# JohannesBuchner/massivedatans

Measured on AMD Instinct MI355X. Metric: likelihood evals/sec across N datasets per constrained draw, higher is better.
Workload: dtype f64

## Files before the change

### massivedatans_amd/csrc/mdns_core.hip

```cpp
#include "mdns_internal.h"
#include <time.h>

#include <atomic>
#include <cmath>
#include <cstdarg>
#include <cstdio>
#include <cstdlib>
#include <cstring>
#include <mutex>
#include <vector>

namespace mdns {

static char g_error[512] = "";

void set_error(const char *fmt, ...)
{
	va_list ap;
	va_start(ap, fmt);
	vsnprintf(g_error, sizeof(g_error), fmt, ap);
	va_end(ap);
	if (getenv("MDNS_VERBOSE")) fprintf(stderr, "[mdns] %s\n", g_error);
}

// ... 33 lines not shown
	if (device >= count) {
		set_error("device %d requested but only %d visible", device, count);
		return 1;
	}
	if (g_ctx_ready) {
		set_error("mdns_init(%d): this process already runs on device %d; one process drives one GPU "
		          "(start one process per GPU)", device, g_ctx.device);
		return 1;
	}
	if (!MDNS_HIP(hipSetDevice(device))) return 1;
	hipDeviceProp_t prop;
	if (!MDNS_HIP(hipGetDeviceProperties(&prop, device))) return 1;
	g_ctx.device = device;
	g_ctx.num_cus = prop.multiProcessorCount > 0 ? prop.multiProcessorCount : 256;
	if (!MDNS_HIP(hipStreamCreateWithFlags(&g_ctx.own_stream, hipStreamNonBlocking))) return 1;
	g_ctx.stream = g_ctx.own_stream;
	g_ctx_ready = true;
	return 0;
}

Context *ctx()
{
	std::lock_guard<std::mutex> lock(g_ctx_mutex);
	if (!g_ctx_ready && init_locked(-1) != 0) return nullptr;
	(void) hipSetDevice(g_ctx.device);
	return &g_ctx;
}

void *device_scratch(size_t bytes)
{
	Context *c = ctx();
	if (!c) return nullptr;
	if (bytes <= c->d_ws_bytes) return c->d_ws;
	if (c->d_ws) {
		(void) hipStreamSynchronize(c->stream);
		(void) hipFree(c->d_ws);
		c->d_ws = nullptr; c->d_ws_bytes = 0;
	}
	size_t cap = bytes + bytes / 2 + 4096;
	if (!MDNS_HIP(hipMalloc(&c->d_ws, cap))) return nullptr;
	c->d_ws_bytes = cap;
	return c->d_ws;
}

void *mask_scratch(size_t bytes)
{
	Context *c = ctx();
	if (!c) return nullptr;
	if (bytes <= c->d_mask_bytes) return c->d_mask;
	if (c->d_mask) {
		(void) hipStreamSynchronize(c->stream);
		(void) hipFree(c->d_mask);
		c->d_mask = nullptr; c->d_mask_bytes = 0;
	}
	size_t cap = bytes + bytes / 2 + 4096;
	if (!MDNS_HIP(hipMalloc(&c->d_mask, cap))) return nullptr;
	c->d_mask_bytes = cap;
	return c->d_mask;
}

void *pinned_scratch(size_t bytes)
{
	Context *c = ctx();
	if (!c) return nullptr;
	if (bytes <= c->h_pin_bytes) return c->h_pin;
// ... 46 lines not shown

static void drain_pending()
{
	for (TimedLaunch &t : g_pending) {
		float ms = 0;
		if (hipEventSynchronize(t.stop) == hipSuccess && hipEventElapsedTime(&ms, t.start, t.stop) == hipSuccess) {
			g_prof_count[t.which] += 1;
			g_prof_ms[t.which] += ms;
		}
		g_event_pool.push_back(t.start);
		g_event_pool.push_back(t.stop);
	}
	g_pending.clear();
}

ProfileScope::ProfileScope(int which) : slot(-1)
{
	if (!(g_profiling & (1 << which)) || !g_ctx_ready) return;
	if (g_prof_seen[which]++ % g_prof_every != 0) return;
	TimedLaunch t{which, pooled_event(), pooled_event()};
	if (!t.start || !t.stop) return;
	(void) hipEventRecord(t.start, g_ctx.stream);
	g_pending.push_back(t);
	slot = (int) g_pending.size() - 1;
}

ProfileScope::~ProfileScope()
{
	if (slot < 0) return;
	(void) hipEventRecord(g_pending[slot].stop, g_ctx.stream);
	if (g_pending.size() >= 4096) drain_pending();
}

template <typename T>
static bool grow(T **p, size_t *cap, size_t need)
{
	if (need <= *cap) return true;
	Context *c = ctx();
	if (!c) return false;
	if (*p) { (void) hipStreamSynchronize(c->stream); (void) hipFree(*p); *p = nullptr; *cap = 0; }
	size_t n = need + need / 2 + 64;
	if (!MDNS_HIP(hipMalloc((void **) p, n * sizeof(T)))) return false;
	*cap = n;
	return true;
}
// ... 13 lines not shown
}

extern "C" int mdns_init(int device)
{
	std::lock_guard<std::mutex> lock(g_ctx_mutex);
	return init_locked(device);
}

extern "C" void *mdns_dev_alloc(size_t bytes)
{
	if (!ctx()) return nullptr;
	void *p = nullptr;
	if (!MDNS_HIP(hipMalloc(&p, bytes ? bytes : 8))) return nullptr;
	return p;
}
extern "C" void mdns_dev_free(void *p) { if (p && ctx()) (void) hipFree(p); }
extern "C" int mdns_h2d(void *dst, const void *src, size_t bytes)
{
	Context *c = ctx();
	if (!c) return 1;
	if (!MDNS_HIP(hipMemcpyAsync(dst, src, bytes, hipMemcpyHostToDevice, c->stream))) return 1;
	return MDNS_HIP(hipStreamSynchronize(c->stream)) ? 0 : 1;
}
extern "C" int mdns_d2h(void *dst, const void *src, size_t bytes)
{
	Context *c = ctx();
	if (!c) return 1;
	if (!MDNS_HIP(hipMemcpyAsync(dst, src, bytes, hipMemcpyDeviceToHost, c->stream))) return 1;
	return MDNS_HIP(hipStreamSynchronize(c->stream)) ? 0 : 1;
}
extern "C" int mdns_d2d(void *dst, const void *src, size_t bytes)
{
	Context *c = ctx();
	if (!c) return 1;
	return MDNS_HIP(hipMemcpyAsync(dst, src, bytes, hipMemcpyDeviceToDevice, c->stream)) ? 0 : 1;
}
extern "C" int mdns_sync(void)
{
	Context *c = ctx();
	if (!c) return 1;
	return MDNS_HIP(hipStreamSynchronize(c->stream)) ? 0 : 1;
}
extern "C" int mdns_set_stream(void *hip_stream)
{
	Context *c = ctx();
	if (!c) return 1;
	c->stream = hip_stream ? (hipStream_t) hip_stream : c->own_stream;
	return 0;
}
extern "C" void *mdns_get_stream(void)
{
	Context *c = ctx();
	return c ? (void *) c->stream : nullptr;
}
extern "C" void *mdns_event_create(void)
{
	if (!ctx()) return nullptr;
	hipEvent_t ev;
	if (!MDNS_HIP(hipEventCreate(&ev))) return nullptr;
	return (void *) ev;
}
extern "C" void mdns_event_destroy(void *ev) { if (ev) (void) hipEventDestroy((hipEvent_t) ev); }
extern "C" int mdns_event_record(void *ev)
{
	Context *c = ctx();
	if (!c || !ev) return 1;
	return MDNS_HIP(hipEventRecord((hipEvent_t) ev, c->stream)) ? 0 : 1;
}
extern "C" double mdns_event_elapsed_ms(void *a, void *b)
{
	if (!a || !b) return NAN;
	if (!MDNS_HIP(hipEventSynchronize((hipEvent_t) b))) return NAN;
	float ms = 0;
	if (!MDNS_HIP(hipEventElapsedTime(&ms, (hipEvent_t) a, (hipEvent_t) b))) return NAN;
	return (double) ms;
}

extern "C" int mdns_profile(int classes)
{
	if (!ctx()) return 1;
	drain_pending();
// ... 341 lines not shown
	if (temporary) mdns_spectra_destroy(s);
	if (rc != 0) return rc;
	double *Lout = (double *) Loutp;
	for (int k = 0; k < M; k++) Lout[rows[k]] = L[k];
	return 0;
}

extern "C" int mdns_count_within_dev(const double *d_members, int K, int ndim, double maxdistance,
                                     const double *d_cands, int M, int *d_counts)
{
	Context *c = ctx();
	if (!c) return 1;
	if (K < 0 || M < 0 || ndim <= 0) { set_error("mdns_count_within_dev: bad sizes"); return 1; }
	if (M == 0) return 0;
	if (K == 0) return MDNS_HIP(hipMemsetAsync(d_counts, 0, (size_t) M * sizeof(int), c->stream)) ? 0 : 1;
	return launch_count_within(d_members, K, ndim, sqrt_threshold(maxdistance), nullptr, d_cands, M, d_counts) ? 0 : 1;
}

extern "C" int mdns_bootstrap_round_maxsq_dev(const double *d_members, int K, int ndim,
                                              const double *d_chosen, int nbootstraps,
                                              double *d_round_sq)
{
	Context *c = ctx();
	if (!c) return 1;
	if (K < 0 || nbootstraps < 0 || ndim <= 0) { set_error("mdns_bootstrap_round_maxsq_dev: bad sizes"); return 1; }
	if (nbootstraps == 0) return 0;
	if (K == 0) return MDNS_HIP(hipMemsetAsync(d_round_sq, 0, (size_t) nbootstraps * sizeof(double), c->stream)) ? 0 : 1;
	return launch_bootstrap(d_members, K, ndim, d_chosen, nbootstraps, d_round_sq) ? 0 : 1;
}

static bool stage_in(const void *const *src, const size_t *bytes, int n, size_t extra_bytes, char **d_ptrs,
                     char **d_extra)
{
	Context *c = ctx();
	size_t total = 0;
	for (int i = 0; i < n; i++) total += (bytes[i] + 255) & ~(size_t) 255;
	char *base = (char *) device_scratch(total + extra_bytes + 256);
	if (!base) return false;
	size_t off = 0;
	for (int i = 0; i < n; i++) {
		d_ptrs[i] = base + off;
		if (bytes[i] && !MDNS_HIP(hipMemcpyAsync(d_ptrs[i], src[i], bytes[i], hipMemcpyHostToDevice, c->stream)))
			return false;
// ... 145 lines not shown
			void *p = g_pool[i].p;
			g_pool[i] = g_pool.back();
			g_pool.pop_back();
			*got = want;
			return p;
		}
	void *p = nullptr;
	if (!MDNS_HIP(hipMalloc(&p, want))) return nullptr;
	*got = want;
	return p;
}

static void pool_give(void *p, size_t bytes)
{
	if (!p) return;
	if (g_pool.size() >= 64) { (void) hipFree(p); return; }
	g_pool.push_back({bytes, p});
}

static bool pool_fit(void **p, size_t *cap, size_t need)
{
	if (need <= *cap) return true;
	pool_give(*p, *cap);
	*cap = 0;
	*p = pool_take(need, cap);
	return *p != nullptr;
}

static bool region_fetch(mdns_region *r);

static bool poll_expired(long long *started_ns)
{
	static const double limit_s = [] { const char *v = getenv("MDNS_POLL_TIMEOUT_S"); const double t = v ? atof(v) : 120.0; return t > 0 ? t : 120.0; }();
	struct timespec ts;
	clock_gettime(CLOCK_MONOTONIC, &ts);
	const long long now = (long long) ts.tv_sec * 1000000000LL + ts.tv_nsec;
	if (*started_ns == 0) { *started_ns = now; return false; }
	return (double) (now - *started_ns) * 1e-9 > limit_s;
}

Wait mdns::wait_seq(const volatile unsigned long long *at, unsigned long long want, hipError_t *err)
{
	long long started = 0;
	for (unsigned spin = 0; *at != want; spin++) {
		if ((spin & 1023) != 1023) continue;
		const hipError_t e = hipStreamQuery(g_ctx.stream);
		if (e == hipErrorNotReady) {
			if (poll_expired(&started)) return Wait::timeout;
			continue;
		}
		if (e != hipSuccess) {
			if (err) *err = e;
			return Wait::failed;
		}
		if (*at != want) return Wait::empty;
	}
	std::atomic_thread_fence(std::memory_order_acquire);
	return Wait::ok;
}

template <class Choice>
static bool region_launch_radius(mdns_region *r, bool (*launch)(const double *, int, int, const Choice *, int, double *, const BootstrapFinish *),
                                 const Choice *d_choice, int nbootstraps)
{
	const BootstrapFinish fin = {r->d_counter, r->d_res, r->h_res_dev, ++r->seq};
	if (!launch(r->d_members, r->K, r->ndim, d_choice, nbootstraps, r->d_round, &fin)) return false;
	r->on_device = true;
	r->pending = true;
	return true;
}

static mdns_region *region_new(const double *d_members, double *owned, int K, int ndim)
{
	mdns_region *r = new mdns_region();
	r->d_members = d_members; r->owned = owned; r->K = K; r->ndim = ndim;
	r->slot = take_result_slot();
	if (r->slot < 0) { mdns_region_destroy(r); return nullptr; }
	const ResultSlab &slab = g_slabs[r->slot / kSlabSlots];
	const int i = r->slot % kSlabSlots;
	r->d_res = slab.d_res + i;
	r->d_counter = slab.d_counter + i;
// ... 13 lines not shown
	const size_t bytes = (size_t) K * ndim * sizeof(double);
	size_t got = 0;
	double *d = (double *) pool_take(bytes, &got);
	if (!d) return nullptr;
	if (!MDNS_HIP(hipMemcpyAsync(d, members, bytes, hipMemcpyHostToDevice, c->stream)) ||
	    !MDNS_HIP(hipStreamSynchronize(c->stream))) { pool_give(d, got); return nullptr; }
	mdns_region *r = region_new(d, d, K, ndim);
	if (r) r->owned_bytes = got; else pool_give(d, got);
	return r;
}

static mdns_region *create_bootstrapped(const double *members, int K, int ndim, const unsigned *packed, int nbootstraps,
                                        double *radius, bool wait)
{
	Context *c = ctx();
	if (!c) return nullptr;
	if (!members || !packed || (wait && !radius) || K <= 0 || ndim <= 0 || nbootstraps <= 0 || nbootstraps > 16) {
		set_error("mdns_region_create_bootstrapped: bad arguments (K=%d ndim=%d rounds=%d)", K, ndim, nbootstraps);
		return nullptr;
	}
	const size_t mbytes = (size_t) K * ndim * sizeof(double), pbytes = (size_t) K * sizeof(unsigned);
	const size_t poff = (mbytes + 255) & ~(size_t) 255;
	size_t got = 0;
	char *d = (char *) pool_take(poff + pbytes, &got);
	if (!d) return nullptr;
	char *pin = (char *) pinned_scratch(poff + pbytes);
	if (!pin) { pool_give(d, got); return nullptr; }
	memcpy(pin, members, mbytes);
	memcpy(pin + poff, packed, pbytes);
	if (!MDNS_HIP(hipMemcpyAsync(d, pin, poff + pbytes, hipMemcpyHostToDevice, c->stream))) { pool_give(d, got); return nullptr; }
	mdns_region *r = region_new((const double *) d, (double *) d, K, ndim);
	if (!r) { (void) hipStreamSynchronize(c->stream); pool_give(d, got); return nullptr; }
	r->owned_bytes = got;
	if (!region_launch_radius(r, launch_bootstrap_packed, (const unsigned *) (d + poff), nbootstraps)) {
		(void) hipStreamSynchronize(c->stream);
		mdns_region_destroy(r);
		return nullptr;
	}
	if (!wait) return r;
	*radius = mdns_region_radius(r);
	if (*radius != *radius) { mdns_region_destroy(r); return nullptr; }
	return r;
}

extern "C" mdns_region *mdns_region_create_bootstrapped(const double *members, int K, int ndim,
                                                        const unsigned *packed, int nbootstraps, double *radius)
{
	return create_bootstrapped(members, K, ndim, packed, nbootstraps, radius, true);
}

mdns_region *mdns::region_begin_bootstrapped(const double *members, int K, int ndim, const unsigned *packed, int nbootstraps)
{
	return create_bootstrapped(members, K, ndim, packed, nbootstraps, nullptr, false);
}

bool mdns::region_view(mdns_region *r, RegionView *out)
{
	if (!r || !out || !r->on_device) return false;
	out->d_members = r->d_members; out->K = r->K; out->ndim = r->ndim; out->d_res = r->d_res;
	return true;
}

extern "C" mdns_region *mdns_region_wrap_dev(const double *d_members, int K, int ndim)
{
	if (!ctx()) return nullptr;
	if (!d_members || K <= 0 || ndim <= 0) { set_error("mdns_region_wrap_dev: bad arguments"); return nullptr; }
	return region_new(d_members, nullptr, K, ndim);
}

extern "C" void mdns_region_destroy(mdns_region *r)
{
	if (!r) return;
	if (r->pending && ctx()) (void) region_fetch(r);
	pool_give(r->owned, r->owned_bytes);
	pool_give(r->own_round, r->own_round_bytes);
	pool_give(r->d_chosen, r->chosen_bytes);
	pool_give(r->d_points, r->points_bytes);
	pool_give(r->d_counts, r->counts_bytes);
	if (r->slot >= 0) g_free_slots.push_back(r->slot);
	delete r;
}

extern "C" int mdns_region_set_radius(mdns_region *r, double maxdistance)
{
	if (!r) { set_error("null region"); return 1; }
	if (r->pending && ctx()) (void) region_fetch(r);
	r->radius = maxdistance;
	r->thresh_sq = sqrt_threshold(maxdistance);
	r->on_device = false;
	r->pending = false;
	return 0;
}

static bool region_fetch(mdns_region *r)
{
	if (!r->pending) return true;
	hipError_t e = hipSuccess;
	switch (wait_seq(&r->h_res->seq, r->seq, &e)) {
	case Wait::ok: break;
	case Wait::timeout: set_error("radius computation: no result within MDNS_POLL_TIMEOUT_S"); return false;
	case Wait::failed: set_error("radius computation failed: %s", hipGetErrorString(e)); return false;
	case Wait::empty: set_error("radius computation finished without a result"); return false;
	}
	r->radius = r->h_res->radius;
	r->thresh_sq = sqrt_threshold(r->radius);
	r->pending = false;
	return true;
}

extern "C" double mdns_region_radius(mdns_region *r)
{
	if (!r || !ctx() || !region_fetch(r)) return NAN;
	return r->radius;
}

extern "C" int mdns_region_bootstrap_radius_async(mdns_region *r, const double *d_chosen, int nbootstraps)
{
	Context *c = ctx();
	if (!c || !r) return 1;
	if (nbootstraps <= 0) { set_error("mdns_region_bootstrap_radius: nbootstraps=%d", nbootstraps); return 1; }
	if (!region_fetch(r)) return 1;
	if (r->round_cap < nbootstraps) {
		if (!pool_fit((void **) &r->own_round, &r->own_round_bytes, (size_t) nbootstraps * sizeof(double))) return 1;
		r->d_round = r->own_round;
		if (!MDNS_HIP(hipMemsetAsync(r->d_round, 0, (size_t) nbootstraps * sizeof(double), c->stream))) return 1;
		r->round_cap = nbootstraps;
	}
	return region_launch_radius(r, launch_bootstrap, d_chosen, nbootstraps) ? 0 : 1;
}

extern "C" double mdns_region_bootstrap_radius_dev(mdns_region *r, const double *d_chosen, int nbootstraps)
{
	if (mdns_region_bootstrap_radius_async(r, d_chosen, nbootstraps) != 0) return NAN;
	return mdns_region_radius(r);
}

extern "C" double mdns_region_bootstrap_radius(mdns_region *r, const double *chosen, int nbootstraps)
{
	Context *c = ctx();
	if (!c || !r) return NAN;
	const size_t n = (size_t) r->K * (nbootstraps > 0 ? nbootstraps : 0);
	if (n == 0) { set_error("mdns_region_bootstrap_radius: nbootstraps=%d", nbootstraps); return NAN; }
	if (!pool_fit(&r->d_chosen, &r->chosen_bytes, n * sizeof(double))) return NAN;
	if (!MDNS_HIP(hipMemcpyAsync(r->d_chosen, chosen, n * sizeof(double), hipMemcpyHostToDevice, c->stream))) return NAN;
	return mdns_region_bootstrap_radius_dev(r, (const double *) r->d_chosen, nbootstraps);
}

extern "C" double mdns_region_bootstrap_radius_packed(mdns_region *r, const unsigned *packed, int nbootstraps)
{
	Context *c = ctx();
	if (!c || !r) return NAN;
	if (nbootstraps <= 0 || nbootstraps > 16 || !packed) { set_error("mdns_region_bootstrap_radius_packed: nbootstraps=%d (1..16)", nbootstraps); return NAN; }
	if (!region_fetch(r)) return NAN;
	const size_t bytes = (size_t) r->K * sizeof(unsigned);
	if (!pool_fit(&r->d_chosen, &r->chosen_bytes, bytes)) return NAN;
	if (!MDNS_HIP(hipMemcpyAsync(r->d_chosen, packed, bytes, hipMemcpyHostToDevice, c->stream))) return NAN;
	if (!region_launch_radius(r, launch_bootstrap_packed, (const unsigned *) r->d_chosen, nbootstraps)) return NAN;
	return mdns_region_radius(r);
}

extern "C" int mdns_region_count_dev(mdns_region *r, const double *d_points, int M, int *d_counts)
{
	if (!ctx() || !r) return 1;
	if (M < 0) { set_error("mdns_region_count: M=%d", M); return 1; }
	if (M == 0) return 0;
	if (!r->on_device && r->radius != r->radius) { set_error("mdns_region_count: the region has no radius yet"); return 1; }
	return launch_count_within(r->d_members, r->K, r->ndim, r->thresh_sq, r->on_device ? r->d_res : nullptr,
	                           d_points, M, d_counts) ? 0 : 1;
}

static char *g_stage = nullptr, *g_stage_dev = nullptr;
static size_t g_stage_points = 0, g_stage_doubles = 0;
static unsigned long long g_stage_seq = 0;
static int *g_stage_ticket = nullptr;

extern "C" int mdns_region_count_polled(mdns_region *r, const double *points, int M, int *counts)
{
	Context *c = ctx();
	if (!c || !r) return 1;
	if (M <= 0) return M < 0;
	if (!r->on_device && r->radius != r->radius) { set_error("mdns_region_count: the region has no radius yet"); return 1; }
	const size_t n = (size_t) M * r->ndim;
	if ((size_t) M > g_stage_points || n > g_stage_doubles) {
		if (g_stage) { (void) hipStreamSynchronize(c->stream); (void) hipHostFree(g_stage); g_stage = nullptr; }
		const size_t np = (size_t) M + M / 2 + 1024, nd = n + n / 2 + 4096;
		if (!MDNS_HIP(hipHostMalloc((void **) &g_stage, 64 + np * sizeof(int) + 64 + nd * sizeof(double), hipHostMallocMapped)) ||
		    !MDNS_HIP(hipHostGetDevicePointer((void **) &g_stage_dev, g_stage, 0))) { g_stage = nullptr; g_stage_points = g_stage_doubles = 0; return 1; }
		g_stage_points = np; g_stage_doubles = nd;
		*(volatile unsigned long long *) g_stage = g_stage_seq;
	}
	if (!g_stage_ticket) {
		if (!MDNS_HIP(hipMalloc((void **) &g_stage_ticket, sizeof(int))) ||
		    !MDNS_HIP(hipMemsetAsync(g_stage_ticket, 0, sizeof(int), c->stream))) { g_stage_ticket = nullptr; return 1; }
	}
	const size_t off_counts = 64, off_points = (64 + g_stage_points * sizeof(int) + 63) & ~(size_t) 63;
	memcpy(g_stage + off_points, points, n * sizeof(double));
	const unsigned long long seq = ++g_stage_seq;
	const CountMail mail = {g_stage_ticket, (unsigned long long *) g_stage_dev, seq};
	if (!launch_count_within(r->d_members, r->K, r->ndim, r->thresh_sq, r->on_device ? r->d_res : nullptr,
	                         (const double *) (g_stage_dev + off_points), M, (int *) (g_stage_dev + off_counts), &mail)) return 1;
	hipError_t e = hipSuccess;
	switch (wait_seq((const volatile unsigned long long *) g_stage, seq, &e)) {
	case Wait::ok: break;
	case Wait::timeout: set_error("membership count: no result within MDNS_POLL_TIMEOUT_S"); return 1;
	case Wait::failed: set_error("membership count failed: %s", hipGetErrorString(e)); return 1;
	case Wait::empty:
		(void) hipMemsetAsync(g_stage_ticket, 0, sizeof(int), c->stream);
		set_error("membership count finished without a result");
		return 1;
	}
	memcpy(counts, g_stage + off_counts, (size_t) M * sizeof(int));
	return 0;
}

extern "C" int mdns_region_count(mdns_region *r, const double *points, int M, int *counts)
{
	Context *c = ctx();
	if (!c || !r) return 1;
	if (M <= 0) return M < 0;
	const size_t n = (size_t) M * r->ndim;
	if (!pool_fit(&r->d_points, &r->points_bytes, n * sizeof(double)) ||
	    !pool_fit(&r->d_counts, &r->counts_bytes, (size_t) M * sizeof(int))) return 1;
	if (!MDNS_HIP(hipMemcpyAsync(r->d_points, points, n * sizeof(double), hipMemcpyHostToDevice, c->stream))) return 1;
	if (mdns_region_count_dev(r, (const double *) r->d_points, M, (int *) r->d_counts) != 0) return 1;
	if (!MDNS_HIP(hipMemcpyAsync(counts, r->d_counts, (size_t) M * sizeof(int), hipMemcpyDeviceToHost, c->stream))) return 1;
	return MDNS_HIP(hipStreamSynchronize(c->stream)) ? 0 : 1;
}
```

### massivedatans_amd/csrc/mdns_internal.h

```cpp
#pragma once
#include <hip/hip_runtime.h>
#include <cstddef>
#include <cstdint>
#include "mdns.h"

namespace mdns {

void set_error(const char *fmt, ...);
bool hip_ok(hipError_t e, const char *what, const char *file, int line);
#define MDNS_HIP(call) ::mdns::hip_ok((call), #call, __FILE__, __LINE__)
bool launched(const char *name);

enum class Wait { ok, timeout, failed, empty };
Wait wait_seq(const volatile unsigned long long *at, unsigned long long want, hipError_t *err = nullptr);

struct Context {
	int device = -1;
	hipStream_t own_stream = nullptr;
	hipStream_t stream = nullptr;
	int num_cus = 256;
	void *d_ws = nullptr;   size_t d_ws_bytes = 0;
	void *h_pin = nullptr;  size_t h_pin_bytes = 0;
	void *d_mask = nullptr; size_t d_mask_bytes = 0;
};
Context *ctx();
void *device_scratch(size_t bytes);
void *pinned_scratch(size_t bytes);
void *mask_scratch(size_t bytes);

}

struct mdns_spectra {
	int ndata = 0;
	int nx = 0;
	int ld = 0;
	double *d_y = nullptr;
	double *d_yT = nullptr;
	int ldT = 0;
	double *d_w = nullptr;
	double *d_x = nullptr;
// ... 103 lines not shown
	double radius;
	double thresh;
	unsigned long long seq;
	unsigned long long pad;
};
struct BootstrapFinish {
	unsigned *counter;
	RegionResult *d_res;
	RegionResult *h_res;
	unsigned long long seq;
};

mdns_region *region_begin_bootstrapped(const double *members, int K, int ndim, const unsigned *packed, int nbootstraps);

struct CountMail { int *ticket; unsigned long long *seq_at; unsigned long long seq; };
bool launch_count_within(const double *d_members, int K, int ndim, double thresh_sq,
                         const RegionResult *d_res, const double *d_cands, int M, int *d_counts,
                         const CountMail *mail = nullptr);
bool launch_bootstrap(const double *d_members, int K, int ndim, const double *d_chosen,
                      int nbootstraps, double *d_round_sq, const BootstrapFinish *finish = nullptr);
bool launch_bootstrap_packed(const double *d_members, int K, int ndim, const unsigned *d_packed,
                             int nbootstraps, double *d_round_sq, const BootstrapFinish *finish);
bool launch_nn_maxsq(const double *d_members, int K, int ndim, double *d_out);
bool bootstrap_sorted_applies(int K, int ndim, int nbootstraps);
bool launch_bootstrap_sorted(const double *d_members, int K, int ndim, const unsigned *d_packed, int nbootstraps,
                             double *d_round_sq, const BootstrapFinish *finish);

struct RegionView { const double *d_members; int K, ndim; const RegionResult *d_res; };
bool region_view(mdns_region *r, RegionView *out);
static constexpr int kChainMost = 1024;
static constexpr int kChainDim = 8;
struct ChainSpec {
	int n, ndim, nparams, limit, identity;
	double mn[kChainDim], mx[kChainDim];
// ... 4 lines not shown
struct ChainBox {
	unsigned long long seq;
	int nkept, B;
	int counts[kChainMost];
	double params[kChainMost][3];
	double u[kChainMost * kChainDim];
};
bool launch_box_count(const RegionView &rv, const ChainSpec &spec, ChainBox *box_dev, double *d_props, int *d_counts,
                      const CountMail *mail);
bool launch_chain_accept(const mdns_spectra *s, const ChainSpec &spec, const double *d_props, const int *d_counts,
                         ChainBox *box_dev, double scale, const int *d_rows_in, int *d_rows_dev, int M,
                         const double *d_higher, int *d_flags, int stamp, const JointTrail &trail, void *d_header);

struct ProfileScope {
	int slot;
	explicit ProfileScope(int which);
	~ProfileScope();
};
void note_kernel(int which, const char *fmt, ...);

#ifdef __HIPCC__
__device__ __forceinline__ void handover_release()
{
	__builtin_amdgcn_fence(__ATOMIC_RELEASE, "workgroup");
	asm volatile("s_waitcnt vmcnt(0)" ::: "memory");
}
__device__ __forceinline__ void handover_acquire() { __builtin_amdgcn_fence(__ATOMIC_ACQUIRE, "workgroup"); }
template <class T, class V> __device__ __forceinline__ void mail_store(T *at, V v) { __hip_atomic_store(at, (T) v, __ATOMIC_RELAXED, __HIP_MEMORY_SCOPE_SYSTEM); }
__device__ __forceinline__ void mail_raise(unsigned long long *seq_at, unsigned long long seq) { handover_release(); mail_store(seq_at, seq); }

template <int U>
// ... 119 lines not shown
```

### massivedatans_amd/csrc/mdns_neighbors.hip

```cpp
#include "mdns_geom.h"
#include <cstdlib>
#include <cstring>

#pragma clang fp contract(off)

namespace mdns {

static constexpr int kBlock = 256;
static constexpr int kMaxTile = 512;
static constexpr int kRounds = 16;
static constexpr size_t kLdsBudget = 60 * 1024;

template <int SL> struct Geo {
	static constexpr int PTS = 64 / SL;
	static constexpr int NSLICE = 4 * SL;
};

template <typename T>
__device__ __forceinline__ void stage_to_lds(T *__restrict__ dst, const T *__restrict__ src, int count)
{
	constexpr int U = 8;
	for (int base = 0; base < count; base += U * kBlock) {
		T r[U];
#pragma unroll
// ... 253 lines not shown
{
	__shared__ double wmax[4][RT];
	merge_chunks<RT, false>(part, K, ny, blockIdx.x * (kBlock / 4), mask, nb, round_sq, wmax);
	finish_radius(fin, round_sq, nround_all);
}

static int pick_tile(int ndim, size_t per_member_extra, size_t fixed_bytes)
{
	const size_t per = (size_t) ndim * sizeof(double) + per_member_extra;
	if (fixed_bytes + 16 * per > kLdsBudget) return 0;
	size_t n = (kLdsBudget - fixed_bytes) / per;
	if (n > (size_t) kMaxTile) n = kMaxTile;
	return (int) (n & ~(size_t) 15);
}

bool launch_count_within(const double *d_members, int K, int ndim, double thresh_sq,
                         const RegionResult *d_res, const double *d_cands, int M, int *d_counts, const CountMail *mail)
{
	Context *c = ctx();
	const CountMail none = {nullptr, nullptr, 0};
	const CountMail post = mail ? *mail : none;
	const size_t fixed = 4 * 64 * sizeof(int);
	const int tile_n = pick_tile(ndim, 0, fixed);
	if (tile_n <= 0) { set_error("ndim=%d too large for the member tile", ndim); return false; }
	const bool small = (M + 63) / 64 < 2 * c->num_cus;
	const bool fine = mail != nullptr && small;
	const int pts = fine ? 4 : (small ? 16 : 64);
	const int gx = (M + pts - 1) / pts;
	int want = (2 * c->num_cus + gx - 1) / gx;
	int max_split = (K + tile_n - 1) / tile_n;
	int gy = want < max_split ? want : max_split;
	if (mail) gy = 1;
	if (gy < 1) gy = 1;
	if (gy > 65535) gy = 65535;
	int kchunk = (K + gy - 1) / gy;
	kchunk = ((kchunk + tile_n - 1) / tile_n) * tile_n;
	gy = (K + kchunk - 1) / kchunk;
	const int accumulate = gy > 1 ? 1 : 0;
	if (accumulate && !MDNS_HIP(hipMemsetAsync(d_counts, 0, (size_t) M * sizeof(int), c->stream))) return false;
	const size_t lds = (size_t) tile_n * ndim * sizeof(double) + fixed;
	dim3 grid(gx, gy);
	ProfileScope prof(2);
#define COUNT_LAUNCH(D) do { if (fine) hipLaunchKernelGGL((k_count_within<D, 16>), grid, dim3(kBlock), lds, c->stream, \
		d_members, K, ndim, thresh_sq, d_res, d_cands, M, d_counts, kchunk, tile_n, accumulate, post); \
	else if (small) hipLaunchKernelGGL((k_count_within<D, 4>), grid, dim3(kBlock), lds, c->stream, \
		d_members, K, ndim, thresh_sq, d_res, d_cands, M, d_counts, kchunk, tile_n, accumulate, post); \
	else hipLaunchKernelGGL((k_count_within<D, 1>), grid, dim3(kBlock), lds, c->stream, \
		d_members, K, ndim, thresh_sq, d_res, d_cands, M, d_counts, kchunk, tile_n, accumulate, post); } while (0)
	MDNS_DIM_SWITCH(ndim, COUNT_LAUNCH)
#undef COUNT_LAUNCH
	return launched("k_count_within");
}

template <bool NN>
static bool launch_nearest(const double *d_members, int K, int ndim, const double *d_chosen,
                           int nboot, double *d_round_sq, const BootstrapFinish *finish,
                           const unsigned *d_packed = nullptr)
{
	Context *c = ctx();
	const bool small = (K + 63) / 64 < 2 * c->num_cus;
	const size_t fixed = (size_t) 4 * (NN ? 1 : (nboot > 10 ? kRounds : 10)) * (small ? 16 : 64) * sizeof(double);
	const int tile_n = pick_tile(ndim, sizeof(unsigned), fixed);
	if (tile_n <= 0) { set_error("ndim=%d too large for the member tile", ndim); return false; }
	const size_t lds = (size_t) tile_n * ndim * sizeof(double) + fixed + (size_t) tile_n * sizeof(unsigned);
	unsigned *d_mask = const_cast<unsigned *>(d_packed);
	if (!NN && !d_packed) {
		d_mask = (unsigned *) mask_scratch((size_t) K * sizeof(unsigned));
		if (!d_mask) return false;
	}
	const bool fused = !NN && finish && K <= 2048 && !d_packed;
	const int pts = small ? 16 : 64;
	dim3 grid((K + pts - 1) / pts);
	for (int b0 = 0; b0 < nboot; b0 += kRounds) {
		const int nb = nboot - b0 < kRounds ? nboot - b0 : kRounds;
		if (!NN && !fused && !d_packed) {
			const int nthreads = K > nb ? K : nb;
			hipLaunchKernelGGL(k_pack_chosen, dim3((nthreads + kBlock - 1) / kBlock), dim3(kBlock), 0, c->stream,
			                   d_chosen, K, nboot, b0, nb, d_mask, d_round_sq);
			if (!launched("k_pack_chosen")) return false;
		}
		BootstrapFinish fin = {nullptr, nullptr, nullptr, 0};
		if (finish && b0 + kRounds >= nboot) fin = *finish;
		ProfileScope prof(3);
#define NEAR_LAUNCH_R(D, SL, RT) hipLaunchKernelGGL((k_nearest_chosen<D, NN, SL, RT>), grid, dim3(kBlock), lds, c->stream, \
		d_members, K, ndim, d_mask, nb, d_round_sq + b0, tile_n, fin, d_round_sq, nboot, fused ? d_chosen : nullptr, nboot, b0)
#define NEAR_LAUNCH(D) do { \
	if (small) { if (NN || nb <= 10) NEAR_LAUNCH_R(D, 4, 10); else NEAR_LAUNCH_R(D, 4, kRounds); } \
	else       { if (NN || nb <= 10) NEAR_LAUNCH_R(D, 1, 10); else NEAR_LAUNCH_R(D, 1, kRounds); } } while (0)
		MDNS_DIM_SWITCH(ndim, NEAR_LAUNCH)
#undef NEAR_LAUNCH
#undef NEAR_LAUNCH_R
		if (!launched("k_nearest_chosen")) return false;
	}
	return true;
}

bool launch_bootstrap(const double *d_members, int K, int ndim, const double *d_chosen,
                      int nbootstraps, double *d_round_sq, const BootstrapFinish *finish)
{
	return launch_nearest<false>(d_members, K, ndim, d_chosen, nbootstraps, d_round_sq, finish);
}

static int uniform_chunks(int K)
{
	int most = K / 128;
	if (most < 1) most = 1;
	int best = most < 16 ? most : 16;
	static const char *forced = getenv("MDNS_K6_GY");
	if (forced && atoi(forced) > 0) best = atoi(forced) < most ? atoi(forced) : most;
	return best;
}

bool launch_bootstrap_packed(const double *d_members, int K, int ndim, const unsigned *d_packed,
                             int nbootstraps, double *d_round_sq, const BootstrapFinish *finish)
{
// ... 29 lines not shown
			    !MDNS_HIP(hipMemsetAsync(d_tickets, 0, (size_t) cap * sizeof(unsigned), c->stream))) { d_tickets = nullptr; tickets_cap = 0; return false; }
			tickets_cap = cap;
		}
		unsigned *tickets = fold ? d_tickets : nullptr;
#define UNI_LAUNCH(D) do { if (rt == 10) hipLaunchKernelGGL((k_nearest_uniform<D, 10>), grid, dim3(kBlock), lds, c->stream, d_members, K, d_packed, kchunk, tile_n, d_part, tickets, nbootstraps, d_round_sq, *finish, nbootstraps); \
		else hipLaunchKernelGGL((k_nearest_uniform<D, kRounds>), grid, dim3(kBlock), lds, c->stream, d_members, K, d_packed, kchunk, tile_n, d_part, tickets, nbootstraps, d_round_sq, *finish, nbootstraps); } while (0)
		MDNS_DIM5_SWITCH(ndim, UNI_LAUNCH)
#undef UNI_LAUNCH
		if (!launched("k_nearest_uniform")) return false;
		if (fold) return true;
		const dim3 fgrid((K + kBlock / 4 - 1) / (kBlock / 4));
		if (rt == 10) hipLaunchKernelGGL((k_nearest_finish<10>), fgrid, dim3(kBlock), 0, c->stream, (const double *) d_part, K, ny, d_packed, nbootstraps, d_round_sq, *finish, nbootstraps);
		else hipLaunchKernelGGL((k_nearest_finish<kRounds>), fgrid, dim3(kBlock), 0, c->stream, (const double *) d_part, K, ny, d_packed, nbootstraps, d_round_sq, *finish, nbootstraps);
		return launched("k_nearest_finish");
	}
	return launch_nearest<false>(d_members, K, ndim, nullptr, nbootstraps, d_round_sq, finish, d_packed);
}

bool launch_nn_maxsq(const double *d_members, int K, int ndim, double *d_out)
{
	return launch_nearest<true>(d_members, K, ndim, nullptr, 1, d_out, nullptr);
}

}
```

Measured before the change: 28.38 billion.

## Run async region bootstrap and count kernels on a side stream with fork/join events

Adds a second non-blocking stream plus fork/join events so the async region radius bootstrap and device-side count launches can run beside work on the main stream. The fork is skipped when no other context entry happened since the last fork, and every synchronous entry point, copy, free and region access joins the side stream first. The aim is to overlap region kernels with other GPU work and to avoid serialising them behind the main stream. The cost is extra bookkeeping, event waits and new ordering hazards, for example an entry point that forgets to join.

```diff
diff --git a/massivedatans_amd/csrc/mdns_core.hip b/massivedatans_amd/csrc/mdns_core.hip
--- a/massivedatans_amd/csrc/mdns_core.hip
+++ b/massivedatans_amd/csrc/mdns_core.hip
@@ -71,17 +71,46 @@
 	g_ctx.device = device;
 	g_ctx.num_cus = prop.multiProcessorCount > 0 ? prop.multiProcessorCount : 256;
 	if (!MDNS_HIP(hipStreamCreateWithFlags(&g_ctx.own_stream, hipStreamNonBlocking))) return 1;
+	if (!MDNS_HIP(hipStreamCreateWithFlags(&g_ctx.region_stream, hipStreamNonBlocking))) return 1;
+	if (!MDNS_HIP(hipEventCreateWithFlags(&g_ctx.fork_event, hipEventDisableTiming))) return 1;
+	if (!MDNS_HIP(hipEventCreateWithFlags(&g_ctx.join_event, hipEventDisableTiming))) return 1;
 	g_ctx.stream = g_ctx.own_stream;
 	g_ctx_ready = true;
 	return 0;
 }
 
-Context *ctx()
+static Context *ctx_entered(bool counts)
 {
 	std::lock_guard<std::mutex> lock(g_ctx_mutex);
 	if (!g_ctx_ready && init_locked(-1) != 0) return nullptr;
 	(void) hipSetDevice(g_ctx.device);
+	if (counts) g_ctx.entered++;
 	return &g_ctx;
+}
+
+Context *ctx() { return ctx_entered(true); }
+
+static hipStream_t region_fork(Context *c)
+{
+	if (c->stream != c->own_stream) return c->stream;
+	if (c->entered != c->forked_at || c->stream_lent) {
+		if (!MDNS_HIP(hipEventRecord(c->fork_event, c->own_stream)) ||
+		    !MDNS_HIP(hipStreamWaitEvent(c->region_stream, c->fork_event, 0))) return nullptr;
+	}
+	c->region_busy = true;
+	return c->region_stream;
+}
+static void region_forked(Context *c, hipStream_t on) { if (on == c->region_stream) c->forked_at = c->entered; }
+
+bool region_join(Context *c)
+{
+	if (!c->region_busy) return true;
+	c->region_busy = false;
+	return MDNS_HIP(hipEventRecord(c->join_event, c->region_stream)) && MDNS_HIP(hipStreamWaitEvent(c->stream, c->join_event, 0));
+}
+static void region_drain(Context *c)
+{
+	if (c->region_busy) (void) hipStreamSynchronize(c->region_stream);
 }
 
 void *device_scratch(size_t bytes)
@@ -106,6 +135,7 @@
 	if (!c) return nullptr;
 	if (bytes <= c->d_mask_bytes) return c->d_mask;
 	if (c->d_mask) {
+		region_drain(c);
 		(void) hipStreamSynchronize(c->stream);
 		(void) hipFree(c->d_mask);
 		c->d_mask = nullptr; c->d_mask_bytes = 0;
@@ -182,13 +212,13 @@
 	g_pending.clear();
 }
 
-ProfileScope::ProfileScope(int which) : slot(-1)
+ProfileScope::ProfileScope(int which, hipStream_t on_) : slot(-1), on(on_ ? on_ : g_ctx.stream)
 {
 	if (!(g_profiling & (1 << which)) || !g_ctx_ready) return;
 	if (g_prof_seen[which]++ % g_prof_every != 0) return;
 	TimedLaunch t{which, pooled_event(), pooled_event()};
 	if (!t.start || !t.stop) return;
-	(void) hipEventRecord(t.start, g_ctx.stream);
+	(void) hipEventRecord(t.start, on);
 	g_pending.push_back(t);
 	slot = (int) g_pending.size() - 1;
 }
@@ -196,7 +226,7 @@
 ProfileScope::~ProfileScope()
 {
 	if (slot < 0) return;
-	(void) hipEventRecord(g_pending[slot].stop, g_ctx.stream);
+	(void) hipEventRecord(g_pending[slot].stop, on);
 	if (g_pending.size() >= 4096) drain_pending();
 }
 
@@ -240,44 +270,59 @@
 	if (!MDNS_HIP(hipMalloc(&p, bytes ? bytes : 8))) return nullptr;
 	return p;
 }
-extern "C" void mdns_dev_free(void *p) { if (p && ctx()) (void) hipFree(p); }
+extern "C" void mdns_dev_free(void *p)
+{
+	Context *c = p ? ctx() : nullptr;
+	if (!c) return;
+	region_drain(c);
+	(void) hipFree(p);
+}
 extern "C" int mdns_h2d(void *dst, const void *src, size_t bytes)
 {
 	Context *c = ctx();
-	if (!c) return 1;
+	if (!c || !region_join(c)) return 1;
 	if (!MDNS_HIP(hipMemcpyAsync(dst, src, bytes, hipMemcpyHostToDevice, c->stream))) return 1;
 	return MDNS_HIP(hipStreamSynchronize(c->stream)) ? 0 : 1;
 }
 extern "C" int mdns_d2h(void *dst, const void *src, size_t bytes)
 {
 	Context *c = ctx();
-	if (!c) return 1;
+	if (!c || !region_join(c)) return 1;
 	if (!MDNS_HIP(hipMemcpyAsync(dst, src, bytes, hipMemcpyDeviceToHost, c->stream))) return 1;
 	return MDNS_HIP(hipStreamSynchronize(c->stream)) ? 0 : 1;
 }
 extern "C" int mdns_d2d(void *dst, const void *src, size_t bytes)
 {
 	Context *c = ctx();
+	if (!c || !region_join(c)) return 1;
+	return MDNS_HIP(hipMemcpyAsync(dst, src, bytes, hipMemcpyDeviceToDevice, c->stream)) ? 0 : 1;
+}
+extern "C" int mdns_sync(void)
+{
+	Context *c = ctx();
 	if (!c) return 1;
-	return MDNS_HIP(hipMemcpyAsync(dst, src, bytes, hipMemcpyDeviceToDevice, c->stream)) ? 0 : 1;
-}
-extern "C" int mdns_sync(void)
+	if (c->region_busy) {
+		c->region_busy = false;
+		if (!MDNS_HIP(hipStreamSynchronize(c->region_stream))) return 1;
+	}
+	return MDNS_HIP(hipStreamSynchronize(c->stream)) ? 0 : 1;
+}
+extern "C" int mdns_set_stream(void *hip_stream)
 {
 	Context *c = ctx();
 	if (!c) return 1;
-	return MDNS_HIP(hipStreamSynchronize(c->stream)) ? 0 : 1;
-}
-extern "C" int mdns_set_stream(void *hip_stream)
-{
-	Context *c = ctx();
-	if (!c) return 1;
+	const bool busy = c->region_busy;
+	if (!region_join(c)) return 1;
 	c->stream = hip_stream ? (hipStream_t) hip_stream : c->own_stream;
+	if (busy && !MDNS_HIP(hipStreamWaitEvent(c->stream, c->join_event, 0))) return 1;
 	return 0;
 }
 extern "C" void *mdns_get_stream(void)
 {
 	Context *c = ctx();
-	return c ? (void *) c->stream : nullptr;
+	if (!c) return nullptr;
+	if (c->stream == c->own_stream) c->stream_lent = true;
+	return (void *) c->stream;
 }
 extern "C" void *mdns_event_create(void)
 {
@@ -290,7 +335,7 @@
 extern "C" int mdns_event_record(void *ev)
 {
 	Context *c = ctx();
-	if (!c || !ev) return 1;
+	if (!c || !ev || !region_join(c)) return 1;
 	return MDNS_HIP(hipEventRecord((hipEvent_t) ev, c->stream)) ? 0 : 1;
 }
 extern "C" double mdns_event_elapsed_ms(void *a, void *b)
@@ -662,7 +707,7 @@
 	if (K < 0 || M < 0 || ndim <= 0) { set_error("mdns_count_within_dev: bad sizes"); return 1; }
 	if (M == 0) return 0;
 	if (K == 0) return MDNS_HIP(hipMemsetAsync(d_counts, 0, (size_t) M * sizeof(int), c->stream)) ? 0 : 1;
-	return launch_count_within(d_members, K, ndim, sqrt_threshold(maxdistance), nullptr, d_cands, M, d_counts) ? 0 : 1;
+	return launch_count_within(c->stream, d_members, K, ndim, sqrt_threshold(maxdistance), nullptr, d_cands, M, d_counts) ? 0 : 1;
 }
 
 extern "C" int mdns_bootstrap_round_maxsq_dev(const double *d_members, int K, int ndim,
@@ -673,8 +718,9 @@
 	if (!c) return 1;
 	if (K < 0 || nbootstraps < 0 || ndim <= 0) { set_error("mdns_bootstrap_round_maxsq_dev: bad sizes"); return 1; }
 	if (nbootstraps == 0) return 0;
+	if (!region_join(c)) return 1;
 	if (K == 0) return MDNS_HIP(hipMemsetAsync(d_round_sq, 0, (size_t) nbootstraps * sizeof(double), c->stream)) ? 0 : 1;
-	return launch_bootstrap(d_members, K, ndim, d_chosen, nbootstraps, d_round_sq) ? 0 : 1;
+	return launch_bootstrap(c->stream, d_members, K, ndim, d_chosen, nbootstraps, d_round_sq) ? 0 : 1;
 }
 
 static bool stage_in(const void *const *src, const size_t *bytes, int n, size_t extra_bytes, char **d_ptrs,
@@ -850,6 +896,7 @@
 static void pool_give(void *p, size_t bytes)
 {
 	if (!p) return;
+	if (g_ctx.region_busy) (void) region_join(&g_ctx);
 	if (g_pool.size() >= 64) { (void) hipFree(p); return; }
 	g_pool.push_back({bytes, p});
 }
@@ -880,7 +927,8 @@
 	long long started = 0;
 	for (unsigned spin = 0; *at != want; spin++) {
 		if ((spin & 1023) != 1023) continue;
-		const hipError_t e = hipStreamQuery(g_ctx.stream);
+		hipError_t e = hipStreamQuery(g_ctx.stream);
+		if (e == hipSuccess && g_ctx.region_busy) e = hipStreamQuery(g_ctx.region_stream);
 		if (e == hipErrorNotReady) {
 			if (poll_expired(&started)) return Wait::timeout;
 			continue;
@@ -895,12 +943,11 @@
 	return Wait::ok;
 }
 
-template <class Choice>
-static bool region_launch_radius(mdns_region *r, bool (*launch)(const double *, int, int, const Choice *, int, double *, const BootstrapFinish *),
-                                 const Choice *d_choice, int nbootstraps)
+template <class Launch>
+static bool region_launch_radius(mdns_region *r, Launch launch)
 {
 	const BootstrapFinish fin = {r->d_counter, r->d_res, r->h_res_dev, ++r->seq};
-	if (!launch(r->d_members, r->K, r->ndim, d_choice, nbootstraps, r->d_round, &fin)) return false;
+	if (!launch(&fin)) return false;
 	r->on_device = true;
 	r->pending = true;
 	return true;
@@ -944,7 +991,7 @@
                                         double *radius, bool wait)
 {
 	Context *c = ctx();
-	if (!c) return nullptr;
+	if (!c || !region_join(c)) return nullptr;
 	if (!members || !packed || (wait && !radius) || K <= 0 || ndim <= 0 || nbootstraps <= 0 || nbootstraps > 16) {
 		set_error("mdns_region_create_bootstrapped: bad arguments (K=%d ndim=%d rounds=%d)", K, ndim, nbootstraps);
 		return nullptr;
@@ -962,7 +1009,8 @@
 	mdns_region *r = region_new((const double *) d, (double *) d, K, ndim);
 	if (!r) { (void) hipStreamSynchronize(c->stream); pool_give(d, got); return nullptr; }
 	r->owned_bytes = got;
-	if (!region_launch_radius(r, launch_bootstrap_packed, (const unsigned *) (d + poff), nbootstraps)) {
+	if (!region_launch_radius(r, [&](const BootstrapFinish *fin) {
+		    return launch_bootstrap_packed(r->d_members, K, ndim, (const unsigned *) (d + poff), nbootstraps, r->d_round, fin); })) {
 		(void) hipStreamSynchronize(c->stream);
 		mdns_region_destroy(r);
 		return nullptr;
@@ -987,6 +1035,7 @@
 bool mdns::region_view(mdns_region *r, RegionView *out)
 {
 	if (!r || !out || !r->on_device) return false;
+	if (!region_join(&g_ctx)) return false;
 	out->d_members = r->d_members; out->K = r->K; out->ndim = r->ndim; out->d_res = r->d_res;
 	return true;
 }
@@ -1002,6 +1051,7 @@
 {
 	if (!r) return;
 	if (r->pending && ctx()) (void) region_fetch(r);
+	if (g_ctx_ready) (void) region_join(&g_ctx);
 	pool_give(r->owned, r->owned_bytes);
 	pool_give(r->own_round, r->own_round_bytes);
 	pool_give(r->d_chosen, r->chosen_bytes);
@@ -1015,6 +1065,7 @@
 {
 	if (!r) { set_error("null region"); return 1; }
 	if (r->pending && ctx()) (void) region_fetch(r);
+	if (g_ctx_ready && !region_join(&g_ctx)) return 1;
 	r->radius = maxdistance;
 	r->thresh_sq = sqrt_threshold(maxdistance);
 	r->on_device = false;
@@ -1044,31 +1095,42 @@
 	return r->radius;
 }
 
-extern "C" int mdns_region_bootstrap_radius_async(mdns_region *r, const double *d_chosen, int nbootstraps)
-{
-	Context *c = ctx();
-	if (!c || !r) return 1;
+static int region_radius_launch(Context *c, mdns_region *r, const double *d_chosen, int nbootstraps, bool beside)
+{
 	if (nbootstraps <= 0) { set_error("mdns_region_bootstrap_radius: nbootstraps=%d", nbootstraps); return 1; }
 	if (!region_fetch(r)) return 1;
+	if (r->round_cap < nbootstraps && !pool_fit((void **) &r->own_round, &r->own_round_bytes, (size_t) nbootstraps * sizeof(double))) return 1;
+	const hipStream_t on = beside ? region_fork(c) : (region_join(c) ? c->stream : nullptr);
+	if (!on) return 1;
 	if (r->round_cap < nbootstraps) {
-		if (!pool_fit((void **) &r->own_round, &r->own_round_bytes, (size_t) nbootstraps * sizeof(double))) return 1;
 		r->d_round = r->own_round;
-		if (!MDNS_HIP(hipMemsetAsync(r->d_round, 0, (size_t) nbootstraps * sizeof(double), c->stream))) return 1;
+		if (!MDNS_HIP(hipMemsetAsync(r->d_round, 0, (size_t) nbootstraps * sizeof(double), on))) return 1;
 		r->round_cap = nbootstraps;
 	}
-	return region_launch_radius(r, launch_bootstrap, d_chosen, nbootstraps) ? 0 : 1;
+	const bool ok = region_launch_radius(r, [&](const BootstrapFinish *fin) {
+		return launch_bootstrap(on, r->d_members, r->K, r->ndim, d_chosen, nbootstraps, r->d_round, fin); });
+	region_forked(c, on);
+	return ok ? 0 : 1;
+}
+
+extern "C" int mdns_region_bootstrap_radius_async(mdns_region *r, const double *d_chosen, int nbootstraps)
+{
+	Context *c = ctx_entered(false);
+	if (!c || !r) return 1;
+	return region_radius_launch(c, r, d_chosen, nbootstraps, true);
 }
 
 extern "C" double mdns_region_bootstrap_radius_dev(mdns_region *r, const double *d_chosen, int nbootstraps)
 {
-	if (mdns_region_bootstrap_radius_async(r, d_chosen, nbootstraps) != 0) return NAN;
+	Context *c = ctx();
+	if (!c || !r || region_radius_launch(c, r, d_chosen, nbootstraps, false) != 0) return NAN;
 	return mdns_region_radius(r);
 }
 
 extern "C" double mdns_region_bootstrap_radius(mdns_region *r, const double *chosen, int nbootstraps)
 {
 	Context *c = ctx();
-	if (!c || !r) return NAN;
+	if (!c || !r || !region_join(c)) return NAN;
 	const size_t n = (size_t) r->K * (nbootstraps > 0 ? nbootstraps : 0);
 	if (n == 0) { set_error("mdns_region_bootstrap_radius: nbootstraps=%d", nbootstraps); return NAN; }
 	if (!pool_fit(&r->d_chosen, &r->chosen_bytes, n * sizeof(double))) return NAN;
@@ -1081,22 +1143,33 @@
 	Context *c = ctx();
 	if (!c || !r) return NAN;
 	if (nbootstraps <= 0 || nbootstraps > 16 || !packed) { set_error("mdns_region_bootstrap_radius_packed: nbootstraps=%d (1..16)", nbootstraps); return NAN; }
-	if (!region_fetch(r)) return NAN;
+	if (!region_fetch(r) || !region_join(c)) return NAN;
 	const size_t bytes = (size_t) r->K * sizeof(unsigned);
 	if (!pool_fit(&r->d_chosen, &r->chosen_bytes, bytes)) return NAN;
 	if (!MDNS_HIP(hipMemcpyAsync(r->d_chosen, packed, bytes, hipMemcpyHostToDevice, c->stream))) return NAN;
-	if (!region_launch_radius(r, launch_bootstrap_packed, (const unsigned *) r->d_chosen, nbootstraps)) return NAN;
+	if (!region_launch_radius(r, [&](const BootstrapFinish *fin) {
+		    return launch_bootstrap_packed(r->d_members, r->K, r->ndim, (const unsigned *) r->d_chosen, nbootstraps, r->d_round, fin); })) return NAN;
 	return mdns_region_radius(r);
 }
 
-extern "C" int mdns_region_count_dev(mdns_region *r, const double *d_points, int M, int *d_counts)
-{
-	if (!ctx() || !r) return 1;
+static int region_count_launch(Context *c, mdns_region *r, const double *d_points, int M, int *d_counts, bool beside)
+{
 	if (M < 0) { set_error("mdns_region_count: M=%d", M); return 1; }
 	if (M == 0) return 0;
 	if (!r->on_device && r->radius != r->radius) { set_error("mdns_region_count: the region has no radius yet"); return 1; }
-	return launch_count_within(r->d_members, r->K, r->ndim, r->thresh_sq, r->on_device ? r->d_res : nullptr,
-	                           d_points, M, d_counts) ? 0 : 1;
+	const hipStream_t on = beside ? region_fork(c) : (region_join(c) ? c->stream : nullptr);
+	if (!on) return 1;
+	const bool ok = launch_count_within(on, r->d_members, r->K, r->ndim, r->thresh_sq, r->on_device ? r->d_res : nullptr,
+	                                    d_points, M, d_counts);
+	region_forked(c, on);
+	return ok ? 0 : 1;
+}
+
+extern "C" int mdns_region_count_dev(mdns_region *r, const double *d_points, int M, int *d_counts)
+{
+	Context *c = ctx_entered(false);
+	if (!c || !r) return 1;
+	return region_count_launch(c, r, d_points, M, d_counts, true);
 }
 
 static char *g_stage = nullptr, *g_stage_dev = nullptr;
@@ -1107,7 +1180,7 @@
 extern "C" int mdns_region_count_polled(mdns_region *r, const double *points, int M, int *counts)
 {
 	Context *c = ctx();
-	if (!c || !r) return 1;
+	if (!c || !r || !region_join(c)) return 1;
 	if (M <= 0) return M < 0;
 	if (!r->on_device && r->radius != r->radius) { set_error("mdns_region_count: the region has no radius yet"); return 1; }
 	const size_t n = (size_t) M * r->ndim;
@@ -1127,7 +1200,7 @@
 	memcpy(g_stage + off_points, points, n * sizeof(double));
 	const unsigned long long seq = ++g_stage_seq;
 	const CountMail mail = {g_stage_ticket, (unsigned long long *) g_stage_dev, seq};
-	if (!launch_count_within(r->d_members, r->K, r->ndim, r->thresh_sq, r->on_device ? r->d_res : nullptr,
+	if (!launch_count_within(c->stream, r->d_members, r->K, r->ndim, r->thresh_sq, r->on_device ? r->d_res : nullptr,
 	                         (const double *) (g_stage_dev + off_points), M, (int *) (g_stage_dev + off_counts), &mail)) return 1;
 	hipError_t e = hipSuccess;
 	switch (wait_seq((const volatile unsigned long long *) g_stage, seq, &e)) {
@@ -1146,13 +1219,13 @@
 extern "C" int mdns_region_count(mdns_region *r, const double *points, int M, int *counts)
 {
 	Context *c = ctx();
-	if (!c || !r) return 1;
+	if (!c || !r || !region_join(c)) return 1;
 	if (M <= 0) return M < 0;
 	const size_t n = (size_t) M * r->ndim;
 	if (!pool_fit(&r->d_points, &r->points_bytes, n * sizeof(double)) ||
 	    !pool_fit(&r->d_counts, &r->counts_bytes, (size_t) M * sizeof(int))) return 1;
 	if (!MDNS_HIP(hipMemcpyAsync(r->d_points, points, n * sizeof(double), hipMemcpyHostToDevice, c->stream))) return 1;
-	if (mdns_region_count_dev(r, (const double *) r->d_points, M, (int *) r->d_counts) != 0) return 1;
+	if (region_count_launch(c, r, (const double *) r->d_points, M, (int *) r->d_counts, false) != 0) return 1;
 	if (!MDNS_HIP(hipMemcpyAsync(counts, r->d_counts, (size_t) M * sizeof(int), hipMemcpyDeviceToHost, c->stream))) return 1;
 	return MDNS_HIP(hipStreamSynchronize(c->stream)) ? 0 : 1;
 }
diff --git a/massivedatans_amd/csrc/mdns_internal.h b/massivedatans_amd/csrc/mdns_internal.h
--- a/massivedatans_amd/csrc/mdns_internal.h
+++ b/massivedatans_amd/csrc/mdns_internal.h
@@ -18,12 +18,19 @@
 	int device = -1;
 	hipStream_t own_stream = nullptr;
 	hipStream_t stream = nullptr;
+	hipStream_t region_stream = nullptr;
+	hipEvent_t fork_event = nullptr, join_event = nullptr;
+	bool region_busy = false;
+	unsigned long long entered = 0;
+	unsigned long long forked_at = 0;
+	bool stream_lent = false;
 	int num_cus = 256;
 	void *d_ws = nullptr;   size_t d_ws_bytes = 0;
 	void *h_pin = nullptr;  size_t h_pin_bytes = 0;
 	void *d_mask = nullptr; size_t d_mask_bytes = 0;
 };
 Context *ctx();
+bool region_join(Context *c);
 void *device_scratch(size_t bytes);
 void *pinned_scratch(size_t bytes);
 void *mask_scratch(size_t bytes);
@@ -157,10 +164,10 @@
 mdns_region *region_begin_bootstrapped(const double *members, int K, int ndim, const unsigned *packed, int nbootstraps);
 
 struct CountMail { int *ticket; unsigned long long *seq_at; unsigned long long seq; };
-bool launch_count_within(const double *d_members, int K, int ndim, double thresh_sq,
+bool launch_count_within(hipStream_t on, const double *d_members, int K, int ndim, double thresh_sq,
                          const RegionResult *d_res, const double *d_cands, int M, int *d_counts,
                          const CountMail *mail = nullptr);
-bool launch_bootstrap(const double *d_members, int K, int ndim, const double *d_chosen,
+bool launch_bootstrap(hipStream_t on, const double *d_members, int K, int ndim, const double *d_chosen,
                       int nbootstraps, double *d_round_sq, const BootstrapFinish *finish = nullptr);
 bool launch_bootstrap_packed(const double *d_members, int K, int ndim, const unsigned *d_packed,
                              int nbootstraps, double *d_round_sq, const BootstrapFinish *finish);
@@ -195,7 +202,8 @@
 
 struct ProfileScope {
 	int slot;
-	explicit ProfileScope(int which);
+	hipStream_t on;
+	explicit ProfileScope(int which, hipStream_t on = nullptr);
 	~ProfileScope();
 };
 void note_kernel(int which, const char *fmt, ...);
diff --git a/massivedatans_amd/csrc/mdns_neighbors.hip b/massivedatans_amd/csrc/mdns_neighbors.hip
--- a/massivedatans_amd/csrc/mdns_neighbors.hip
+++ b/massivedatans_amd/csrc/mdns_neighbors.hip
@@ -291,7 +291,7 @@
 	return (int) (n & ~(size_t) 15);
 }
 
-bool launch_count_within(const double *d_members, int K, int ndim, double thresh_sq,
+bool launch_count_within(hipStream_t on, const double *d_members, int K, int ndim, double thresh_sq,
                          const RegionResult *d_res, const double *d_cands, int M, int *d_counts, const CountMail *mail)
 {
 	Context *c = ctx();
@@ -314,15 +314,15 @@
 	kchunk = ((kchunk + tile_n - 1) / tile_n) * tile_n;
 	gy = (K + kchunk - 1) / kchunk;
 	const int accumulate = gy > 1 ? 1 : 0;
-	if (accumulate && !MDNS_HIP(hipMemsetAsync(d_counts, 0, (size_t) M * sizeof(int), c->stream))) return false;
+	if (accumulate && !MDNS_HIP(hipMemsetAsync(d_counts, 0, (size_t) M * sizeof(int), on))) return false;
 	const size_t lds = (size_t) tile_n * ndim * sizeof(double) + fixed;
 	dim3 grid(gx, gy);
-	ProfileScope prof(2);
-#define COUNT_LAUNCH(D) do { if (fine) hipLaunchKernelGGL((k_count_within<D, 16>), grid, dim3(kBlock), lds, c->stream, \
+	ProfileScope prof(2, on);
+#define COUNT_LAUNCH(D) do { if (fine) hipLaunchKernelGGL((k_count_within<D, 16>), grid, dim3(kBlock), lds, on, \
 		d_members, K, ndim, thresh_sq, d_res, d_cands, M, d_counts, kchunk, tile_n, accumulate, post); \
-	else if (small) hipLaunchKernelGGL((k_count_within<D, 4>), grid, dim3(kBlock), lds, c->stream, \
+	else if (small) hipLaunchKernelGGL((k_count_within<D, 4>), grid, dim3(kBlock), lds, on, \
 		d_members, K, ndim, thresh_sq, d_res, d_cands, M, d_counts, kchunk, tile_n, accumulate, post); \
-	else hipLaunchKernelGGL((k_count_within<D, 1>), grid, dim3(kBlock), lds, c->stream, \
+	else hipLaunchKernelGGL((k_count_within<D, 1>), grid, dim3(kBlock), lds, on, \
 		d_members, K, ndim, thresh_sq, d_res, d_cands, M, d_counts, kchunk, tile_n, accumulate, post); } while (0)
 	MDNS_DIM_SWITCH(ndim, COUNT_LAUNCH)
 #undef COUNT_LAUNCH
@@ -330,7 +330,7 @@
 }
 
 template <bool NN>
-static bool launch_nearest(const double *d_members, int K, int ndim, const double *d_chosen,
+static bool launch_nearest(hipStream_t on, const double *d_members, int K, int ndim, const double *d_chosen,
                            int nboot, double *d_round_sq, const BootstrapFinish *finish,
                            const unsigned *d_packed = nullptr)
 {
@@ -352,14 +352,14 @@
 		const int nb = nboot - b0 < kRounds ? nboot - b0 : kRounds;
 		if (!NN && !fused && !d_packed) {
 			const int nthreads = K > nb ? K : nb;
-			hipLaunchKernelGGL(k_pack_chosen, dim3((nthreads + kBlock - 1) / kBlock), dim3(kBlock), 0, c->stream,
+			hipLaunchKernelGGL(k_pack_chosen, dim3((nthreads + kBlock - 1) / kBlock), dim3(kBlock), 0, on,
 			                   d_chosen, K, nboot, b0, nb, d_mask, d_round_sq);
 			if (!launched("k_pack_chosen")) return false;
 		}
 		BootstrapFinish fin = {nullptr, nullptr, nullptr, 0};
 		if (finish && b0 + kRounds >= nboot) fin = *finish;
-		ProfileScope prof(3);
-#define NEAR_LAUNCH_R(D, SL, RT) hipLaunchKernelGGL((k_nearest_chosen<D, NN, SL, RT>), grid, dim3(kBlock), lds, c->stream, \
+		ProfileScope prof(3, on);
+#define NEAR_LAUNCH_R(D, SL, RT) hipLaunchKernelGGL((k_nearest_chosen<D, NN, SL, RT>), grid, dim3(kBlock), lds, on, \
 		d_members, K, ndim, d_mask, nb, d_round_sq + b0, tile_n, fin, d_round_sq, nboot, fused ? d_chosen : nullptr, nboot, b0)
 #define NEAR_LAUNCH(D) do { \
 	if (small) { if (NN || nb <= 10) NEAR_LAUNCH_R(D, 4, 10); else NEAR_LAUNCH_R(D, 4, kRounds); } \
@@ -372,10 +372,10 @@
 	return true;
 }
 
-bool launch_bootstrap(const double *d_members, int K, int ndim, const double *d_chosen,
+bool launch_bootstrap(hipStream_t on, const double *d_members, int K, int ndim, const double *d_chosen,
                       int nbootstraps, double *d_round_sq, const BootstrapFinish *finish)
 {
-	return launch_nearest<false>(d_members, K, ndim, d_chosen, nbootstraps, d_round_sq, finish);
+	return launch_nearest<false>(on, d_members, K, ndim, d_chosen, nbootstraps, d_round_sq, finish);
 }
 
 static int uniform_chunks(int K)
@@ -435,12 +435,13 @@
 		else hipLaunchKernelGGL((k_nearest_finish<kRounds>), fgrid, dim3(kBlock), 0, c->stream, (const double *) d_part, K, ny, d_packed, nbootstraps, d_round_sq, *finish, nbootstraps);
 		return launched("k_nearest_finish");
 	}
-	return launch_nearest<false>(d_members, K, ndim, nullptr, nbootstraps, d_round_sq, finish, d_packed);
+	return launch_nearest<false>(c->stream, d_members, K, ndim, nullptr, nbootstraps, d_round_sq, finish, d_packed);
 }
 
 bool launch_nn_maxsq(const double *d_members, int K, int ndim, double *d_out)
 {
-	return launch_nearest<true>(d_members, K, ndim, nullptr, 1, d_out, nullptr);
-}
-
-}
+	Context *c = ctx();
+	return launch_nearest<true>(c->stream, d_members, K, ndim, nullptr, 1, d_out, nullptr);
+}
+
+}
```

Result: slower. 23.59 billion (-16.9%).
